# lh3/miniasm

Measured on AMD Instinct MI355X. Metric: PAF overlaps processed/sec (hit-filter->trans-reduce->GFA), higher is better.
Workload: dtype u32

## Files before the change

include/mahip.h:

```cpp
#ifndef MAHIP_H
#define MAHIP_H

#include <stddef.h>
#include <stdint.h>
#include "miniasm_amd.h"

#ifdef __cplusplus
extern "C" {
#endif

typedef struct mahip_ctx mahip_ctx_t;

int mahip_device_count(void);
mahip_ctx_t *mahip_create(int device, void *stream);
void mahip_destroy(mahip_ctx_t *c);
const char *mahip_strerror(void);
int mahip_sync(mahip_ctx_t *c);
int mahip_first_launch(mahip_ctx_t *c);

int mahip_hits_upload(mahip_ctx_t *c, const ma_hit_t *h, size_t n, uint32_t n_seq);
int mahip_hits_adopt(mahip_ctx_t *c, const void *d_hits, size_t n, uint32_t n_seq);
int mahip_set_shard(mahip_ctx_t *c, uint32_t q_beg, uint32_t q_end);
int mahip_hits_balance(mahip_ctx_t *c, int world, uint32_t *bounds);
int mahip_set_shard_bounds(mahip_ctx_t *c, const uint32_t *bounds, int world);
const uint32_t *mahip_shard_bounds(mahip_ctx_t *c, int *world);

typedef struct {
	uint64_t n_lines;
	uint64_t n_records;
	uint64_t n_stored_lines;
	uint64_t n_hits;
	uint64_t name_bytes;
	uint32_t n_seq, max_qs;
	uint32_t n_excl;
} mahip_paf_info_t;
int mahip_paf_load_mem(mahip_ctx_t *c, const void *text, size_t nbytes);
int mahip_paf_load_fd(mahip_ctx_t *c, int fd, size_t nbytes);
int mahip_paf_parse(mahip_ctx_t *c, int min_span, int min_match, int bi_dir, mahip_paf_info_t *info);
int mahip_paf_parse_excl(mahip_ctx_t *c, int min_span, int min_match, int bi_dir, int no_cont, int max_hang, float int_frac, mahip_paf_info_t *info);
int mahip_paf_load_fd_range(mahip_ctx_t *c, int fd, size_t off, size_t nbytes);
int mahip_paf_parse_sharded(mahip_ctx_t *c, int min_span, int min_match, int bi_dir, mahip_paf_info_t *info);
int mahip_hits_route(mahip_ctx_t *c, uint64_t *n_total, uint64_t *bytes_sent);
int mahip_paf_names(mahip_ctx_t *c, char *names, uint32_t *lens);
int mahip_paf_seqs(mahip_ctx_t *c, char *names, void *seqs16, uint64_t *tot_len);
int mahip_paf_release(mahip_ctx_t *c);
uint32_t mahip_paf_max_qs(mahip_ctx_t *c);
int mahip_hits_raw_download(mahip_ctx_t *c, ma_hit_t *out);
int mahip_hits_raw_extract(mahip_ctx_t *c, uint32_t q_beg, uint32_t q_end, void *d_dst, size_t *n_out);
int mahip_hits_raw_extract_pos(mahip_ctx_t *c, uint32_t q_beg, uint32_t q_end, void *d_dst, uint32_t *d_pos, size_t *n_out);
int mahip_hits_set_positions(mahip_ctx_t *c, const uint32_t *pos, int on_device, uint64_t n_total);
int mahip_hits_have_positions(mahip_ctx_t *c);

int mahip_set_hints(mahip_ctx_t *c, uint32_t max_qs);
int mahip_set_run_stride(mahip_ctx_t *c, int stride);
uint64_t mahip_hits_sorted_runs(mahip_ctx_t *c);
int mahip_memcpy_h2d(mahip_ctx_t *c, void *d_dst, const void *h_src, size_t bytes);
int mahip_memcpy_d2h(mahip_ctx_t *c, void *h_dst, const void *d_src, size_t bytes);
int mahip_set_exact_ties(mahip_ctx_t *c, int mode);
typedef struct {
	uint64_t arc_tie_groups;
	uint64_t arc_tie_arcs;
	uint64_t push_conflicts;
	uint64_t hit_ties;
	int arc_walk, hit_walk;
	int unrepaired;
	uint64_t push_conflicts_seen;
	uint64_t hit_walk_reads;
} mahip_tie_info_t;
int mahip_tie_stats(mahip_ctx_t *c, mahip_tie_info_t *out);
int mahip_hits_sort(mahip_ctx_t *c);
int mahip_hits_index(mahip_ctx_t *c);

int mahip_hits_sub(mahip_ctx_t *c, int min_dp, float min_iden, int end_clip, int slot, size_t *n_remained);
int mahip_hits_cut(mahip_ctx_t *c, int slot, int min_span, size_t *n_live);
int mahip_hits_flt(mahip_ctx_t *c, int slot, int max_hang, int min_ovlp, size_t *n_live, float *cov);
int mahip_sub_merge(mahip_ctx_t *c);
int mahip_hits_contained(mahip_ctx_t *c, const ma_opt_t *opt, const uint8_t *seq_del, uint32_t *n_seq_new, size_t *n_live);

int mahip_hits_cutflt_sub(mahip_ctx_t *c, int cut_slot, int min_span, int max_hang, int min_ovlp, int min_dp, float min_iden, int end_clip,
                          int out_slot, size_t *n_cut, size_t *n_flt, float *cov, size_t *n_remained);
int mahip_hits_cut_contained(mahip_ctx_t *c, int cut_slot, int min_span, const ma_opt_t *opt, size_t *n_cut, uint32_t *n_seq_new);
int mahip_hits_cut_contained_flags(mahip_ctx_t *c, int cut_slot, int min_span, const ma_opt_t *opt);
int mahip_hits_cut_contained_finish(mahip_ctx_t *c, size_t *n_cut, uint32_t *n_seq_new);

int mahip_sub_upload(mahip_ctx_t *c, int slot, const ma_sub_t *sub, size_t n_sub);
int mahip_sub_download(mahip_ctx_t *c, int slot, ma_sub_t *sub, int squeezed);
int mahip_seqdel_download(mahip_ctx_t *c, uint8_t *del);
int mahip_map_download(mahip_ctx_t *c, int32_t *map);
uint32_t mahip_n_seq_new(mahip_ctx_t *c);
int mahip_survivors_download(mahip_ctx_t *c, uint32_t *old_ids);
size_t mahip_hits_live(mahip_ctx_t *c);
int mahip_hits_download(mahip_ctx_t *c, ma_hit_t *out, size_t *n);

int mahip_sg_gen(mahip_ctx_t *c, const ma_opt_t *opt, int use_sub, const uint32_t *seq_len, const uint8_t *seq_del, uint32_t *n_arc);
int mahip_asg_upload(mahip_ctx_t *c, const asg_t *g);
int mahip_asg_del_trans(mahip_ctx_t *c, int fuzz, uint32_t *n_reduced);
int mahip_asg_symm(mahip_ctx_t *c, uint32_t *n_multi, uint32_t *n_asymm);
int mahip_asg_del_multi(mahip_ctx_t *c, uint32_t *n_multi);
int mahip_asg_del_asymm(mahip_ctx_t *c, uint32_t *n_asymm);
int mahip_asg_del_short(mahip_ctx_t *c, float drop_ratio, uint32_t *n_short);
int mahip_asg_squeeze(mahip_ctx_t *c);
int mahip_tail_handoff(mahip_ctx_t *from, mahip_ctx_t *to);
int mahip_asg_cut_tip(mahip_ctx_t *c, int max_ext, uint32_t *n_cut);
int mahip_asg_cut_internal(mahip_ctx_t *c, int max_ext, uint32_t *n_cut);
int mahip_asg_cut_biloop(mahip_ctx_t *c, int max_ext, uint32_t *n_cut);
int mahip_asg_pop_bubble(mahip_ctx_t *c, int max_dist, uint32_t *n_pop, uint32_t *n_tips);
uint32_t mahip_bubble_seq_sweeps(mahip_ctx_t *c);
int mahip_ug_gen(mahip_ctx_t *c, uint32_t *n_utg, uint32_t *n_members, uint32_t *n_uarc);
int mahip_ug_download(mahip_ctx_t *c, uint32_t *u_n, uint32_t *u_len, uint32_t *u_start, uint32_t *u_end, uint32_t *u_off, uint64_t *members, asg_arc_t *uarcs);
typedef struct { uint64_t src_off, dst_off; uint32_t src_len, len; uint32_t rev, pad; } mahip_useq_job_t;
int mahip_useq_begin(mahip_ctx_t *c, size_t arena_bytes);
int mahip_useq_batch(mahip_ctx_t *c, const char *h_seq, size_t seq_bytes, const mahip_useq_job_t *h_jobs, size_t n_jobs);
int mahip_useq_end(mahip_ctx_t *c, char *h_arena);
uint32_t mahip_asg_n_arc(mahip_ctx_t *c);
uint64_t mahip_asg_trans_inner(mahip_ctx_t *c);
int mahip_asg_download(mahip_ctx_t *c, asg_t *g);

#define MAHIP_BUF_SUB0  0
#define MAHIP_BUF_SUB1  1
#define MAHIP_BUF_RCONT 2
#define MAHIP_BUF_RUSED 3
#define MAHIP_BUF_SDEL  4
int mahip_copy_out(mahip_ctx_t *c, int which, void *d_dst, size_t first, size_t count);
int mahip_copy_in(mahip_ctx_t *c, int which, const void *d_src, size_t first, size_t count);
int mahip_hits_contained_flags(mahip_ctx_t *c, const ma_opt_t *opt);
int mahip_hits_contained_finish(mahip_ctx_t *c, const uint8_t *seq_del, uint32_t *n_seq_new, size_t *n_live);
int mahip_sg_flags(mahip_ctx_t *c, const ma_opt_t *opt, int use_sub, const uint32_t *seq_len, const uint8_t *seq_del);
int mahip_sg_finish(mahip_ctx_t *c, uint32_t *n_arc);
int mahip_asg_export_rows(mahip_ctx_t *c, void *d_dst);
int mahip_asg_import_rows(mahip_ctx_t *c, const void *d_src, const uint32_t *counts, int n_ranks, size_t stride);
int mahip_set_full_input(mahip_ctx_t *c, int full);
int mahip_sg_push_conflicts(mahip_ctx_t *c, uint64_t *n_conf);
int mahip_sg_push_fix(mahip_ctx_t *c);
int mahip_asg_export_rows_push(mahip_ctx_t *c, void *d_dst);
int mahip_asg_import_push_rows(mahip_ctx_t *c, const void *d_src, const uint32_t *counts, int n_ranks, size_t stride);
int mahip_asg_del_trans_range(mahip_ctx_t *c, int fuzz, uint32_t v_beg, uint32_t v_end, uint32_t *n_reduced);
int mahip_asg_flags_out(mahip_ctx_t *c, void *d_dst, size_t first, size_t count);
int mahip_asg_flags_in(mahip_ctx_t *c, const void *d_src, size_t first, size_t count);
int mahip_asg_cleanup(mahip_ctx_t *c, uint32_t *n_arc);

int mahip_comm_unique_id(void *id128);
int mahip_comm_init(mahip_ctx_t *c, const void *id128, int rank, int world);
int mahip_comm_init_shm(mahip_ctx_t *c, const char *name, int rank, int world);
void mahip_comm_destroy(mahip_ctx_t *c);
int mahip_comm_rank(mahip_ctx_t *c);
int mahip_comm_world(mahip_ctx_t *c);
int mahip_comm_active(mahip_ctx_t *c);
int mahip_comm_all_gather(mahip_ctx_t *c, const void *d_send, void *d_recv, size_t bytes_per_rank);
int mahip_comm_all_reduce_max_u8(mahip_ctx_t *c, void *d_buf, size_t n);
int mahip_comm_all_reduce_sum_u64(mahip_ctx_t *c, uint64_t *h_vals, size_t n);
typedef struct {
	void *user;
	int (*all_gather)(void *user, const void *send, void *recv, size_t bytes);
	int (*all_reduce_max_u8)(void *user, void *buf, size_t n);
	int (*all_reduce_sum_u64)(void *user, uint64_t *vals, size_t n);
	int (*all_reduce_sum_u32)(void *user, void *buf, size_t n);
	int (*all_to_all_v)(void *user, const void *send, void *recv, const uint64_t *bytes);
} mahip_comm_ext_t;
int mahip_comm_init_ext(mahip_ctx_t *c, int rank, int world, const mahip_comm_ext_t *ext);
int mahip_comm_all_reduce_sum_u32(mahip_ctx_t *c, void *d_buf, size_t n);
int mahip_comm_all_to_all_v(mahip_ctx_t *c, const void *d_send, void *d_recv, const uint64_t *bytes);
int mahip_comm_all_gather_u64(mahip_ctx_t *c, const uint64_t *h_vals, size_t n, uint64_t *h_out);
int mahip_comm_barrier(mahip_ctx_t *c);
int mahip_xbuf(mahip_ctx_t *c, int slot, size_t bytes, void **d_ptr);

int mahip_prof_enable(mahip_ctx_t *c, int enable);
int mahip_prof_reset(mahip_ctx_t *c);
typedef struct { const char *name; uint64_t launches; double total_ms; double alg_bytes; } mahip_prof_t;
int mahip_prof_get(mahip_ctx_t *c, mahip_prof_t *out, int max);
int mahip_mark(mahip_ctx_t *c, int slot);
int mahip_marks_ms(mahip_ctx_t *c, int first, int n, float *ms);
size_t mahip_mem_bytes(mahip_ctx_t *c);
size_t mahip_mem_pool_bytes(mahip_ctx_t *c);
int mahip_mem_trim(mahip_ctx_t *c, size_t *released);

int mahip_diag_patterns(void);
const char *mahip_diag_name(int pattern);
int mahip_diag_run(mahip_ctx_t *c, int pattern, size_t bytes, int reps, double *best_ms, double *moved);
#define MAHIP_PTR_SUB0    0
#define MAHIP_PTR_SUB1    1
#define MAHIP_PTR_RDFLAG  2
void *mahip_devptr(mahip_ctx_t *c, int which, size_t *bytes);

#ifdef __cplusplus
}
#endif
#endif
```

miniasm_amd/csrc/graph.hip:

```cpp
#include "mahip_internal.hpp"
#include <type_traits>

#define DEAD 0x80000000u
#define ADEL 0x80000000u

struct HitColsG { const uint32_t *qid, *qs, *qe, *tn, *ts, *te, *ml, *bl; };
struct ArcCols { uint32_t *u, *v, *len, *ol; };

static HitColsG gcols_of(mahip_ctx *c)
{
	HitColsG h;
	h.qid = P<uint32_t>(c->col[0]); h.qs = P<uint32_t>(c->col[1]); h.qe = P<uint32_t>(c->col[2]); h.tn = P<uint32_t>(c->col[3]);
	h.ts = P<uint32_t>(c->col[4]); h.te = P<uint32_t>(c->col[5]); h.ml = P<uint32_t>(c->col[6]); h.bl = P<uint32_t>(c->col[7]);
	return h;
}
static ArcCols arcs_of(mahip_ctx *c, int g)
{
	ArcCols a;
	a.u = P<uint32_t>(c->au[g]); a.v = P<uint32_t>(c->av[g]); a.len = P<uint32_t>(c->alen[g]); a.ol = P<uint32_t>(c->aol[g]);
	return a;
}
static int reserve_arcs(mahip_ctx *c, size_t n)
{
	for (int g = 0; g < 2; ++g) {
		CHK(dev_reserve(c, c->au[g], (n + 4) * 4)); CHK(dev_reserve(c, c->av[g], (n + 4) * 4));
		CHK(dev_reserve(c, c->alen[g], (n + 4) * 4)); CHK(dev_reserve(c, c->aol[g], (n + 4) * 4));
	}
	CHK(dev_reserve(c, c->keep, (n + 16) * 4)); CHK(dev_reserve(c, c->pos, (n + 16) * 4));
	return 0;
}

__global__ __launch_bounds__(256) void k_sg_seq(const uint2 *__restrict__ sub, const uint8_t *__restrict__ r_del, const uint32_t *__restrict__ seq_len,
                                                 const uint8_t *__restrict__ seq_del, uint32_t n_seq, uint32_t *__restrict__ slen, uint8_t *__restrict__ sdel)
{
	uint32_t r = blockIdx.x * 256 + threadIdx.x;
	if (r >= n_seq) return;
	uint32_t len; int del;
	if (sub) { uint2 s = sub[r]; len = s.y - (s.x & 0x7fffffffu); del = s.x >> 31; }
	else len = seq_len[r], del = 0;
	if (seq_del) del |= seq_del[r];
	if (r_del) del |= r_del[r];
	slen[r] = len; sdel[r] = (uint8_t)del;
}

#define SG_TILE 16384u

__device__ __forceinline__ int sg_candidate(const HitColsG &h, size_t i, const uint32_t *__restrict__ slen, int max_hang, float int_frac, int min_ovlp,
                                            const uint8_t *__restrict__ lazy_del, mc_arc_t *x, uint32_t *q_, uint32_t *t_, int *self_rc)
{
	const uint32_t q = h.qid[i];
	if (lazy_del && lazy_del[q]) return -100;
	if (h.bl[i] & DEAD) return -100;
	const uint32_t t = h.tn[i];
	if (lazy_del && lazy_del[t]) return -100;
	uint32_t qs = h.qs[i], qe = h.qe[i], ts = h.ts[i], te = h.te[i];
	int rev = h.ml[i] >> 31;
	*q_ = q; *t_ = t;
	*self_rc = q == t && qs == ts && qe == te && rev;
	return mc_hit2arc(q, qs, qe, t, ts, te, rev, (int)slen[q], (int)slen[t], max_hang, int_frac, min_ovlp, x);
}

__global__ __launch_bounds__(256) void k_sg_arcs(HitColsG h, size_t n, const uint32_t *__restrict__ slen, uint8_t *__restrict__ sdel,
                                                  int max_hang, float int_frac, int min_ovlp, unsigned long long *__restrict__ ctr, const uint8_t *__restrict__ lazy_del,
                                                  unsigned long long *__restrict__ cmask)
{
	uint32_t mx = 0, n_live = 0;
	for (size_t base = (size_t)blockIdx.x * 256; base < n; base += (size_t)gridDim.x * 256) {
		const size_t i = base + threadIdx.x;
		int cand = 0;
		if (i < n) {
			mc_arc_t x;
			uint32_t q = 0, t = 0;
			int self_rc = 0, r = sg_candidate(h, i, slen, max_hang, int_frac, min_ovlp, lazy_del, &x, &q, &t, &self_rc);
			if (r != -100) {
				++n_live;
				if (r >= 0) {
					if (q == t) { if (self_rc) sdel[q] = 1; }
					else cand = 1, mx = x.len > mx ? x.len : mx;
				} else if (r == MC_HT_QCONT) sdel[q] = 1;
			}
		}
		const unsigned long long m = wv_ballot(cand);
		if ((threadIdx.x & 63) == 0) cmask[i >> 6] = m;
	}
	blk_max_u64(&ctr[CT_MAXLEN], mx);
	blk_add_u64(&ctr[CT_LIVE], n_live);
}

#ifndef SG_DENSE
#define SG_DENSE 6
#endif
__device__ __forceinline__ unsigned long long wv_bcast_u64(unsigned long long x, int src) { return (unsigned long long)__shfl((uint32_t)(x >> 32), src, 64) << 32 | __shfl((uint32_t)x, src, 64); }

__global__ __launch_bounds__(256) void k_sg_emit(HitColsG h, size_t n, const uint32_t *__restrict__ slen, const uint8_t *__restrict__ sdel,
                                                  int max_hang, float int_frac, int min_ovlp, const unsigned long long *cmask,
                                                  uint32_t *__restrict__ tile_cnt, const uint32_t *__restrict__ tile_off, ArcCols out, uint32_t *__restrict__ aslot,
                                                  uint32_t *__restrict__ wpos, unsigned long long *kmask)
{
	__shared__ uint32_t s_w[4];
	const unsigned lane = threadIdx.x & 63;
	const size_t w = (size_t)blockIdx.x * 256 + threadIdx.x, n_words = (n + 63) >> 6, w0 = w - lane;
	unsigned long long m = w < n_words ? cmask[w] : 0ull, kept = 0;
	uint32_t cnt = 0;
	const bool dense = __popcll(m) >= SG_DENSE;
	const unsigned long long dense_lanes = wv_ballot(dense);
	for (unsigned long long dl = dense_lanes; dl; dl &= dl - 1) {
		const int l = __ffsll((long long)dl) - 1;
		const unsigned long long ml = wv_bcast_u64(m, l);
		const size_t i = ((w0 + (size_t)l) << 6) + lane;
		const int k = (ml >> lane & 1ull) && i < n && !sdel[h.qid[i]] && !sdel[h.tn[i]];
		const unsigned long long kb = wv_ballot(k);
		if ((int)lane == l) kept = kb, cnt = (uint32_t)__popcll(kb);
	}
	if (!dense)
		for (unsigned long long rest = m; rest; rest &= rest - 1) {
			const int b = __ffsll((long long)rest) - 1;
			const size_t i = (w << 6) + (size_t)b;
			if (i < n && !sdel[h.qid[i]] && !sdel[h.tn[i]]) kept |= 1ull << b, ++cnt;
		}
	uint32_t tot, ex = block_excl_scan_256(cnt, s_w, &tot);
	if (!out.u) { if (threadIdx.x == 0) tile_cnt[blockIdx.x] = tot; return; }
	uint32_t p = tile_off[blockIdx.x] + ex;
	if (wpos && w < n_words) { wpos[w] = p; kmask[w] = kept; }
	for (unsigned long long dl = dense_lanes; dl; dl &= dl - 1) {
		const int l = __ffsll((long long)dl) - 1;
		const unsigned long long kl = wv_bcast_u64(kept, l);
		const uint32_t pl = __shfl(p, l, 64);
		if (kl >> lane & 1ull) {
			const size_t i = ((w0 + (size_t)l) << 6) + lane;
			const uint32_t pp = pl + (uint32_t)__popcll(kl & wv_lt(lane));
			mc_arc_t x;
			uint32_t q = 0, t = 0;
			int self_rc = 0;
			sg_candidate(h, i, slen, max_hang, int_frac, min_ovlp, nullptr, &x, &q, &t, &self_rc);
			out.u[pp] = x.u; out.v[pp] = x.v; out.len[pp] = x.len; out.ol[pp] = x.ol;
			if (aslot) aslot[pp] = (uint32_t)i;
		}
	}
	if (!dense)
		for (; kept; kept &= kept - 1, ++p) {
			const size_t i = (w << 6) + (size_t)(__ffsll((long long)kept) - 1);
			mc_arc_t x;
			uint32_t q = 0, t = 0;
			int self_rc = 0;
			sg_candidate(h, i, slen, max_hang, int_frac, min_ovlp, nullptr, &x, &q, &t, &self_rc);
			out.u[p] = x.u; out.v[p] = x.v; out.len[p] = x.len; out.ol[p] = x.ol;
			if (aslot) aslot[p] = (uint32_t)i;
		}
}

__global__ __launch_bounds__(256) void k_arc_keep(ArcCols a, size_t n, const uint8_t *__restrict__ sdel, uint32_t *__restrict__ keep, int use_keep_in)
{
	size_t i = (size_t)blockIdx.x * 256 + threadIdx.x;
	if (i >= n) return;
	int k = use_keep_in ? (int)keep[i] : 1;
	if (k) k = !(a.ol[i] & ADEL) && !sdel[a.u[i] >> 1] && !sdel[a.v[i] >> 1];
	keep[i] = k;
}

__global__ __launch_bounds__(256) void k_arc_compact(ArcCols in, size_t n, const uint32_t *__restrict__ keep, const uint32_t *__restrict__ pos, ArcCols out)
{
	size_t i = (size_t)blockIdx.x * 256 + threadIdx.x;
	if (i < n && keep[i]) {
		uint32_t p = pos[i];
		out.u[p] = in.u[i]; out.v[p] = in.v[i]; out.len[p] = in.len[i]; out.ol[p] = in.ol[i];
	}
}

#define RM_ITEMS 8
#define RM_TILE (256 * RM_ITEMS)
#define RMC_ITEMS 8
#define RMC_TILE (256 * RMC_ITEMS)
#define RMC_TILES 16u
#define RMC_GROUP ((size_t)RMC_TILES * RMC_TILE)
__global__ __launch_bounds__(256) void k_arc_rm_count(const uint32_t *__restrict__ aol, size_t n, uint32_t *__restrict__ cnt)
{
	__shared__ uint32_t s_wave[4];
	const size_t g0 = (size_t)blockIdx.x * RMC_GROUP, g1 = g0 + RMC_GROUP < n ? g0 + RMC_GROUP : n;
	uint32_t mine = 0;
	for (size_t b0 = g0; b0 < g1; b0 += 8 * 1024) {
		uint4 w[8];
#pragma unroll
		for (int j = 0; j < 8; ++j) { const size_t b4 = b0 + (size_t)j * 1024 + (size_t)threadIdx.x * 4; w[j] = b4 + 4 <= g1 ? *(const uint4*)(aol + b4) : make_uint4(ADEL, ADEL, ADEL, ADEL); }
#pragma unroll
		for (int j = 0; j < 8; ++j) {
			const size_t b4 = b0 + (size_t)j * 1024 + (size_t)threadIdx.x * 4;
			mine += !(w[j].x & ADEL) + !(w[j].y & ADEL) + !(w[j].z & ADEL) + !(w[j].w & ADEL);
			if (b4 < g1 && b4 + 4 > g1) for (size_t i = b4; i < g1; ++i) mine += !(aol[i] & ADEL);
		}
	}
	uint32_t gtot;
	(void)block_excl_scan_256(mine, s_wave, &gtot);
	if (threadIdx.x == 0) cnt[blockIdx.x] = gtot;
}
__global__ __launch_bounds__(256) void k_arc_rm_write(ArcCols in, size_t n, ArcCols out, const uint32_t *__restrict__ pre)
{
	__shared__ uint32_t s_wave[4];
	const size_t g0 = (size_t)blockIdx.x * RMC_GROUP, g1 = g0 + RMC_GROUP < n ? g0 + RMC_GROUP : n;
	uint32_t p0 = pre[blockIdx.x];
	for (size_t tb = g0; tb < g1; tb += RMC_TILE) {
		const size_t base = tb + (size_t)threadIdx.x * RMC_ITEMS;
		uint32_t ol[RMC_ITEMS], keep = 0;
		if (base + RMC_ITEMS <= n) {
			const uint4 *po = (const uint4*)(in.ol + base);
			const uint4 c0 = po[0], c1 = po[1];
			ol[0] = c0.x, ol[1] = c0.y, ol[2] = c0.z, ol[3] = c0.w, ol[4] = c1.x, ol[5] = c1.y, ol[6] = c1.z, ol[7] = c1.w;
		} else {
#pragma unroll
			for (int i = 0; i < RMC_ITEMS; ++i) ol[i] = base + i < n ? in.ol[base + i] : ADEL;
		}
#pragma unroll
		for (int i = 0; i < RMC_ITEMS; ++i) if (!(ol[i] & ADEL)) keep |= 1u << i;
		uint32_t tot;
		const uint32_t ex = block_excl_scan_256((uint32_t)__popc(keep), s_wave, &tot);
		uint32_t p = p0 + ex;
#pragma unroll
		for (int i = 0; i < RMC_ITEMS; ++i)
			if (keep >> i & 1u) { out.u[p] = in.u[base + i]; out.v[p] = in.v[base + i]; out.len[p] = in.len[base + i]; out.ol[p] = ol[i]; ++p; }
		p0 += tot;
	}
}

__global__ __launch_bounds__(256) void k_arc_rm_chain(ArcCols in, size_t n, const uint8_t *__restrict__ sdel, ArcCols out, uint32_t *__restrict__ d_total,
                                                       unsigned long long *state, uint32_t *ticket, uint32_t ticket_base, uint32_t epoch)
{
	__shared__ uint32_t s_wave[4];
	__shared__ uint32_t s_tile, s_prefix;
	if (threadIdx.x == 0) s_tile = atomicAdd(ticket, 1u) - ticket_base;
	__syncthreads();
	const uint32_t tile = s_tile;
	const size_t base = (size_t)tile * RM_TILE + (size_t)threadIdx.x * RM_ITEMS;
	uint32_t u[RM_ITEMS], v[RM_ITEMS], ol[RM_ITEMS], keep = 0;
	if (base + RM_ITEMS <= n) {
		const uint4 *pu = (const uint4*)(in.u + base), *pv = (const uint4*)(in.v + base), *po = (const uint4*)(in.ol + base);
		const uint4 a0 = pu[0], a1 = pu[1], b0 = pv[0], b1 = pv[1], c0 = po[0], c1 = po[1];
		u[0] = a0.x, u[1] = a0.y, u[2] = a0.z, u[3] = a0.w, u[4] = a1.x, u[5] = a1.y, u[6] = a1.z, u[7] = a1.w;
// ... 540 lines not shown
				if (mark[y] == 2) aol[st + i] |= ADEL, ++cnt;
				mark[y] = 0;
			}
			if (cnt) atomicAdd(&ctr[CT_NRED], (unsigned long long)cnt);
		}
		__syncthreads();
	}
	blk_add_u64(&ctr[CT_TRINNER], n_inner);
}

__global__ __launch_bounds__(256) void k_asg_multi(ArcCols a, size_t n, const unsigned long long *__restrict__ idx, unsigned long long *__restrict__ ctr)
{
	uint32_t cnt = 0;
	for (size_t e = (size_t)blockIdx.x * 256 + threadIdx.x; e < n; e += (size_t)gridDim.x * 256) {
		uint32_t st = (uint32_t)(idx[a.u[e]] >> 32), v = a.v[e];
		int del = 0;
		for (uint32_t j = st; j < e; ++j) if (a.v[j] == v) { del = 1; break; }
		if (del) a.ol[e] |= ADEL, ++cnt;
	}
	blk_add_u64(&ctr[CT_NMULTI], cnt);
}

__global__ __launch_bounds__(256) void k_asg_asymm(ArcCols a, size_t n, const unsigned long long *__restrict__ idx, unsigned long long *__restrict__ ctr)
{
	uint32_t cnt = 0;
	uint64_t probed = 0;
	for (size_t e = (size_t)blockIdx.x * 256 + threadIdx.x; e < n; e += (size_t)gridDim.x * 256) {
		uint32_t v = a.v[e] ^ 1, u = a.u[e] ^ 1;
		unsigned long long x = idx[v];
		uint32_t st = (uint32_t)(x >> 32), nv = (uint32_t)x, i;
		for (i = 0; i < nv; ++i) if (a.v[st + i] == u) break;
		probed += i < nv ? i + 1 : nv;
		if (i == nv) a.ol[e] |= ADEL, ++cnt;
	}
	blk_add_u64(&ctr[CT_NASYMM], cnt);
	blk_add_u64(&ctr[CT_PROBED], probed);
}

__global__ __launch_bounds__(256) void k_asg_short(ArcCols a, const unsigned long long *__restrict__ idx, uint32_t n_vtx, float drop_ratio, unsigned long long *__restrict__ ctr)
{
	uint32_t cnt = 0;
	for (uint32_t v = blockIdx.x * 256 + threadIdx.x; v < n_vtx; v += gridDim.x * 256) {
		unsigned long long x = idx[v];
		uint32_t st = (uint32_t)(x >> 32), nv = (uint32_t)x;
		if (nv >= 2) {
			float p = (float)(int32_t)(a.ol[st] & 0x7fffffffu) * drop_ratio;
			uint32_t thres = (uint32_t)((double)p + .499), i;
			for (i = nv - 1; i >= 1 && (a.ol[st + i] & 0x7fffffffu) < thres; --i);
			for (i = i + 1; i < nv; ++i) a.ol[st + i] |= ADEL, ++cnt;
		}
	}
	blk_add_u64(&ctr[CT_NSHORT], cnt);
}

__global__ __launch_bounds__(256) void k_arc_from_aos(const asg_arc_t *__restrict__ in, size_t n, ArcCols a)
{
	size_t i = (size_t)blockIdx.x * 256 + threadIdx.x;
	if (i < n) { uint4 r = *(const uint4*)(in + i); a.len[i] = r.x; a.u[i] = r.y; a.v[i] = r.z; a.ol[i] = r.w; }
}
__global__ __launch_bounds__(256) void k_seq_from_aos(const uint32_t *__restrict__ seq, uint32_t n_seq, uint32_t *__restrict__ slen, uint8_t *__restrict__ sdel)
{
	uint32_t r = blockIdx.x * 256 + threadIdx.x;
	if (r < n_seq) { uint32_t x = seq[r]; slen[r] = x & 0x7fffffffu; sdel[r] = (uint8_t)(x >> 31); }
}
__global__ __launch_bounds__(256) void k_arc_to_aos(ArcCols a, size_t n, const int32_t *__restrict__ map, asg_arc_t *__restrict__ out)
{
	size_t i = (size_t)blockIdx.x * 256 + threadIdx.x;
	if (i >= n) return;
	uint32_t u = a.u[i], v = a.v[i];
	if (map) u = (uint32_t)map[u >> 1] << 1 | (u & 1), v = (uint32_t)map[v >> 1] << 1 | (v & 1);
	*(uint4*)(out + i) = make_uint4(a.len[i], u, v, a.ol[i]);
}
__global__ __launch_bounds__(256) void k_seq_to_aos(const uint32_t *__restrict__ slen, const uint8_t *__restrict__ sdel, const unsigned long long *__restrict__ idx,
                                                     const int32_t *__restrict__ map, uint32_t n_seq, uint32_t *__restrict__ seq, unsigned long long *__restrict__ idx_out)
{
	uint32_t r = blockIdx.x * 256 + threadIdx.x;
	if (r >= n_seq) return;
	int32_t m = map ? map[r] : (int32_t)r;
	if (m < 0) return;
	seq[m] = (slen[r] & 0x7fffffffu) | (uint32_t)sdel[r] << 31;
	idx_out[2 * (size_t)m] = idx[2 * (size_t)r]; idx_out[2 * (size_t)m + 1] = idx[2 * (size_t)r + 1];
}


__global__ __launch_bounds__(256) void k_arc_rows_out(ArcCols a, size_t n, uint4 *__restrict__ rows)
{
	size_t i = (size_t)blockIdx.x * 256 + threadIdx.x;
	if (i < n) rows[i] = make_uint4(a.u[i], a.v[i], a.len[i], a.ol[i]);
}
__global__ __launch_bounds__(256) void k_arc_rows_in(const uint4 *__restrict__ rows, size_t n, size_t dst0, ArcCols a)
{
	size_t i = (size_t)blockIdx.x * 256 + threadIdx.x;
	if (i < n) { uint4 r = rows[i]; a.u[dst0 + i] = r.x; a.v[dst0 + i] = r.y; a.len[dst0 + i] = r.z; a.ol[dst0 + i] = r.w; }
}

__global__ __launch_bounds__(256) void k_rows_permute(const uint4 *__restrict__ in, size_t n, const uint32_t *__restrict__ perm, uint4 *__restrict__ out)
{
	size_t i = (size_t)blockIdx.x * 256 + threadIdx.x;
	if (i < n) out[i] = in[perm[i]];
}

uint32_t graph_nseq(const mahip_ctx *c) { return c->gsq ? c->n_seq_new : c->n_seq; }
static const int32_t *graph_map(mahip_ctx *c) { return c->has_map && !c->gsq ? (const int32_t*)P<int32_t>(c->map) : (const int32_t*)nullptr; }

static int arc_reindex(mahip_ctx *c)
{
	size_t V = 2 * (size_t)graph_nseq(c);
	CHK(dev_reserve(c, c->idx, (V + 2) * 8));
	HIPCHK(hipMemsetAsync(c->idx.p, 0, V * 8, c->st));
	if (c->n_arc) {
		ProfScope ps(c, "k_arc_index", 16.0 * (double)c->n_arc);
		hipLaunchKernelGGL(k_arc_index, dim3(grid_for(c->n_arc, 256)), dim3(256), 0, c->st, (const uint32_t*)P<uint32_t>(c->au[c->ag]), (size_t)c->n_arc, P<unsigned long long>(c->idx));
	}
	HIPCHK(hipGetLastError());
	return 0;
}

static int arc_cleanup(mahip_ctx *c, size_t n_in, int keep_in, int index_mode)
{
	uint32_t *d_tot = (uint32_t*)(P<unsigned long long>(c->ctr) + CT_TOTAL);
	if (n_in == 0) { c->n_arc = 0; return index_mode < 0 ? 0 : arc_reindex(c); }
	ArcCols in = arcs_of(c, c->ag), out = arcs_of(c, c->ag ^ 1);
	if (!keep_in) {
		ProfScope ps(c, "k_arc_rm", 32.0 * (double)n_in);
		if (c->arcs_clean) {
			const size_t ng = (n_in + RMC_GROUP - 1) / RMC_GROUP;
			hipLaunchKernelGGL(k_arc_rm_count, dim3((unsigned)ng), dim3(256), 0, c->st, (const uint32_t*)in.ol, n_in, P<uint32_t>(c->keep));
			CHK(scan_exclusive_u32(c, P<uint32_t>(c->keep), P<uint32_t>(c->pos), ng, d_tot));
			hipLaunchKernelGGL(k_arc_rm_write, dim3((unsigned)ng), dim3(256), 0, c->st, in, n_in, out, (const uint32_t*)P<uint32_t>(c->pos));
		} else {
			const size_t nb = (n_in + RM_TILE - 1) / RM_TILE;
			uint32_t *ticket; unsigned long long *state; uint32_t ticket_base, epoch;
			CHK(scan_chain_begin(c, nb, &state, &ticket, &ticket_base, &epoch));
			hipLaunchKernelGGL(k_arc_rm_chain, dim3((unsigned)nb), dim3(256), 0, c->st, in, n_in, (const uint8_t*)P<uint8_t>(c->sdel), out, d_tot, state, ticket, ticket_base, epoch);
		}
	} else {
		ProfScope ps(c, "k_arc_rm", 32.0 * (double)n_in);
		hipLaunchKernelGGL(k_arc_keep, dim3(grid_for(n_in, 256)), dim3(256), 0, c->st, in, n_in, (const uint8_t*)P<uint8_t>(c->sdel), P<uint32_t>(c->keep), keep_in);
		CHK(scan_exclusive_u32(c, P<uint32_t>(c->keep), P<uint32_t>(c->pos), n_in, d_tot));
		hipLaunchKernelGGL(k_arc_compact, dim3(grid_for(n_in, 256)), dim3(256), 0, c->st, in, n_in, (const uint32_t*)P<uint32_t>(c->keep), (const uint32_t*)P<uint32_t>(c->pos), out);
	}
	CHK(ctr_fetch(c));
	uint32_t n_out = (uint32_t)(c->h_ctr[CT_TOTAL] & 0xffffffffu);
	c->ag ^= 1;
	int changed = n_out != n_in;
	c->n_arc = n_out;
	c->arcs_clean = true;
	if (index_mode > 0 || (index_mode == 0 && changed)) CHK(arc_reindex(c));
	return 0;
}

static int bitlen_u64(uint64_t x) { int b = 0; while (x) ++b, x >>= 1; return b; }

extern "C" int mahip_sg_flags(mahip_ctx_t *c, const ma_opt_t *opt, int use_sub, const uint32_t *seq_len, const uint8_t *seq_del)
{
	HIPCHK(hipSetDevice(c->dev));
	CHK(hits_need_cols(c, "mahip_sg_gen"));
	size_t n = c->n_hits;
	uint32_t R = c->n_seq;
	CHK(dev_reserve(c, c->slen, ((size_t)R + 4) * 4)); CHK(dev_reserve(c, c->sdel, (size_t)R + 16));
	c->sg_max_hang = opt->max_hang; c->sg_int_frac = opt->int_frac; c->sg_min_ovlp = opt->min_ovlp;
	c->gsq = false; c->arcs_clean = false;
	CHK(ctr_zero(c));
	unsigned long long *ctr = P<unsigned long long>(c->ctr);
	const uint32_t *d_len = nullptr; const uint8_t *d_del = nullptr;
	if (seq_len) { CHK(dev_reserve(c, c->big0, ((size_t)R + 4) * 4)); HIPCHK(hipMemcpyAsync(c->big0.p, seq_len, (size_t)R * 4, hipMemcpyHostToDevice, c->st)); d_len = P<uint32_t>(c->big0); }
	if (seq_del) { CHK(dev_reserve(c, c->big1, (size_t)R + 16)); HIPCHK(hipMemcpyAsync(c->big1.p, seq_del, R, hipMemcpyHostToDevice, c->st)); d_del = P<uint8_t>(c->big1); }
	if (!use_sub && !d_len) { mahip_set_error("mahip_sg_gen: need sub or seq_len"); return -1; }
	if (R) hipLaunchKernelGGL(k_sg_seq, dim3(grid_for(R, 256)), dim3(256), 0, c->st, use_sub ? (const uint2*)P<uint2>(c->sub[0]) : (const uint2*)nullptr,
	                          c->has_map ? (const uint8_t*)P<uint8_t>(c->r_del) : (const uint8_t*)nullptr, d_len, d_del, R, P<uint32_t>(c->slen), P<uint8_t>(c->sdel));
	c->ag = 0;
	if (n) CHK(dev_reserve(c, c->sgmask, (n / 64 + 8) * 8));
	if (n) {
		ProfScope ps(c, "k_sg_arcs", 64.0 * (double)c->n_live);
		hipLaunchKernelGGL(k_sg_arcs, dim3(grid_for(n, 256, MA_STREAM_BLOCKS)), dim3(256), 0, c->st, gcols_of(c), n, (const uint32_t*)P<uint32_t>(c->slen), P<uint8_t>(c->sdel),
		                   opt->max_hang, opt->int_frac, opt->min_ovlp, ctr,
		                   c->lazy_squeeze ? (const uint8_t*)P<uint8_t>(c->r_del) : (const uint8_t*)nullptr, P<unsigned long long>(c->sgmask));
	}
	HIPCHK(hipGetLastError());
	return 0;
}

static int push_stable_order(mahip_ctx *c, size_t m, int *gen, uint64_t *conflicts)
{
	unsigned long long *ctr = P<unsigned long long>(c->ctr);
	const int bs = hits_qs_bits(c);
	int bq = 0;
	for (uint64_t x = c->n_seq ? c->n_seq - 1 : 0xffffffffull; x; x >>= 1) ++bq;
	for (int k = 0; k < 2; ++k) { CHK(dev_reserve(c, c->key[k], (m + 1) * 8)); CHK(dev_reserve(c, c->val[k], (m + 1) * 4)); }
	hipLaunchKernelGGL(k_arc_slot_keys, dim3(grid_for(m, 256)), dim3(256), 0, c->st, (const uint32_t*)P<uint32_t>(c->aslot), m, c->d_aos, (const uint32_t*)P<uint32_t>(c->sidx),
	                   P<uint64_t>(c->key[0]), P<uint32_t>(c->val[0]));
	*gen = 0;
	CHK(radix_sort_pairs(c, m, 0, bs, 32, 32 + (bq ? bq : 1), gen));
	HIPCHK(hipMemsetAsync(ctr + ST_PUSH_CONFLICTS, 0, 8, c->st));
	hipLaunchKernelGGL(k_arc_push_conflicts, dim3(grid_for(m, 256, MA_STREAM_BLOCKS)), dim3(256), 0, c->st, (const uint64_t*)P<uint64_t>(c->key[*gen]), m, ctr);
	CHK(ctr_fetch(c));
	*conflicts = c->h_ctr[ST_PUSH_CONFLICTS];
	return 0;
}

static int push_order(mahip_ctx *c, size_t m, bool exact, int *gen, const ArcCols *pushed = nullptr, const ArcCols *sorted = nullptr)
{
	uint64_t conf = 0;
	bool want_known = false;
	TieLaps tl(c);
	CHK(push_stable_order(c, m, gen, &conf));
	tl.lap("stable push order + conflicts");
	c->tie.push_conflicts = conf;
	c->tie.push_conflicts_seen = conf;
	static const bool filter_on = !(getenv("MA_TIE_NO_FILTER") && atoi(getenv("MA_TIE_NO_FILTER")) != 0);
	if (exact && conf && pushed && sorted && filter_on && m < 0xffffffffull) {
		unsigned long long *ctr = P<unsigned long long>(c->ctr);
		const int32_t *map = c->has_map ? (const int32_t*)P<int32_t>(c->map) : (const int32_t*)nullptr;
		uint64_t *S = P<uint64_t>(c->key[*gen ^ 1]);
		CHK(dev_reserve(c, c->keep, (m + 16) * 4)); CHK(dev_reserve(c, c->pos, (m + 16) * 4));
		hipLaunchKernelGGL(k_arc_keys_ref, dim3(grid_for(m, 256)), dim3(256), 0, c->st, *sorted, m, map, S);
		hipLaunchKernelGGL(k_tie_pair_flags, dim3(grid_for(m, 256)), dim3(256), 0, c->st, (const uint64_t*)S, m, P<uint32_t>(c->keep));
		CHK(scan_exclusive_u32(c, P<uint32_t>(c->keep), P<uint32_t>(c->pos), m, nullptr));
		HIPCHK(hipMemsetAsync(ctr + ST_PUSH_SEEN, 0, 8, c->st));
		const size_t want_bytes = ((size_t)c->n_seq / 32 + 2) * 4;
		CHK(dev_reserve(c, c->wantb, want_bytes));
		HIPCHK(hipMemsetAsync(c->wantb.p, 0, want_bytes, c->st));
		hipLaunchKernelGGL(k_arc_push_conflicts_seen, dim3(grid_for(m, 256, MA_STREAM_BLOCKS)), dim3(256), 0, c->st, (const uint64_t*)P<uint64_t>(c->key[*gen]), (const uint32_t*)P<uint32_t>(c->val[*gen]),
		                   *pushed, map, (const uint64_t*)S, (const uint32_t*)P<uint32_t>(c->pos), (uint32_t)m, ctr, P<uint32_t>(c->wantb));
		CHK(ctr_fetch(c));
		c->tie.push_conflicts_seen = c->h_ctr[ST_PUSH_SEEN];
		want_known = true;
		tl.lap("conflicts the arc sort can see");
	}
	if (exact && c->tie.push_conflicts_seen) {
		const int g_keep = *gen; (void)g_keep;
		static const bool walk_all = getenv("MA_TIE_WALK_ALL") && atoi(getenv("MA_TIE_WALK_ALL")) != 0;
		CHK(hits_reference_rank(c, false, want_known && !walk_all));
		for (int k = 0; k < 2; ++k) { CHK(dev_reserve(c, c->key[k], (m + 1) * 8)); CHK(dev_reserve(c, c->val[k], (m + 1) * 4)); }
		hipLaunchKernelGGL(k_arc_push_keys, dim3(grid_for(m, 256)), dim3(256), 0, c->st, (const uint32_t*)P<uint32_t>(c->aslot), (const uint32_t*)P<uint32_t>(c->hrank), m,
		                   P<uint64_t>(c->key[0]), P<uint32_t>(c->val[0]));
		*gen = 0;
		int bh = 0;
		for (uint64_t x = c->n_in; x; x >>= 1) ++bh;
		CHK(radix_sort_pairs(c, m, 0, bh ? bh : 1, 0, 0, gen));
	}
	return 0;
}

extern "C" int mahip_sg_finish(mahip_ctx_t *c, uint32_t *n_arc)
{
	HIPCHK(hipSetDevice(c->dev));
	size_t n = c->n_hits;
	uint32_t R = c->n_seq;
	CHK(ctr_fetch(c));
	c->n_live = (size_t)c->h_ctr[CT_LIVE];
	if (c->prof) prof_patch_last(c, "k_sg_arcs", 64.0 * (double)c->n_live);
	c->n_arc = 0; c->ag = 0;
	const bool sharded = c->q_beg > 0 || (c->n_seq && c->q_end < c->n_seq);
	const bool want_slots = c->sorted_here && c->sidx.p != nullptr;
	const int blen = bitlen_u64(c->h_ctr[CT_MAXLEN]);
	{ const uint64_t keep_hit_ties = c->tie.hit_ties; const int keep_walk = c->hrank_ready; memset(&c->tie, 0, sizeof(c->tie)); c->tie.hit_ties = keep_hit_ties; c->tie.hit_walk = keep_walk; }
	if (n) {
		const size_t n_tiles = (n + SG_TILE - 1) / SG_TILE;
		const unsigned long long *lazy = (const unsigned long long*)P<unsigned long long>(c->sgmask);
		uint32_t *d_tot = (uint32_t*)(P<unsigned long long>(c->ctr) + CT_TOTAL);
		ArcCols none = { nullptr, nullptr, nullptr, nullptr };
		CHK(dev_reserve(c, c->keep, (n + 16) * 4)); CHK(dev_reserve(c, c->pos, (n + 16) * 4));
		{
			ProfScope ps(c, "k_sg_emit", 4.0 * (double)n + 64.0 * (double)c->n_live);
			hipLaunchKernelGGL(k_sg_emit, dim3((unsigned)n_tiles), dim3(256), 0, c->st, gcols_of(c), n, (const uint32_t*)P<uint32_t>(c->slen), (const uint8_t*)P<uint8_t>(c->sdel),
			                   c->sg_max_hang, c->sg_int_frac, c->sg_min_ovlp, lazy, P<uint32_t>(c->keep), (const uint32_t*)nullptr, none, (uint32_t*)nullptr, (uint32_t*)nullptr, (unsigned long long*)nullptr);
		}
		CHK(scan_exclusive_u32(c, P<uint32_t>(c->keep), P<uint32_t>(c->pos), n_tiles, d_tot));
		CHK(ctr_fetch(c));
		c->n_arc = (uint32_t)(c->h_ctr[CT_TOTAL] & 0xffffffffu);
		CHK(reserve_arcs(c, c->n_arc));
		if (want_slots) CHK(dev_reserve(c, c->aslot, ((size_t)c->n_arc + 4) * 4));
		CHK(dev_reserve(c, c->apos, (n / 64 + 8) * 4));
		if (c->n_arc) {
			ProfScope ps(c, "k_sg_emit", 4.0 * (double)n + 64.0 * (double)c->n_live + 16.0 * (double)c->n_arc);
			hipLaunchKernelGGL(k_sg_emit, dim3((unsigned)n_tiles), dim3(256), 0, c->st, gcols_of(c), n, (const uint32_t*)P<uint32_t>(c->slen), (const uint8_t*)P<uint8_t>(c->sdel),
			                   c->sg_max_hang, c->sg_int_frac, c->sg_min_ovlp, lazy, (uint32_t*)nullptr, (const uint32_t*)P<uint32_t>(c->pos), arcs_of(c, 0),
			                   want_slots ? P<uint32_t>(c->aslot) : (uint32_t*)nullptr, P<uint32_t>(c->apos), P<unsigned long long>(c->sgmask));
		}
	} else CHK(reserve_arcs(c, 0));
	c->n_push = 0; c->push_ordered = false;
	if (sharded && c->tie_mode != 0) {
		CHK(dev_reserve(c, c->pushrows[0], ((size_t)c->n_arc + 1) * 16));
		if (c->n_arc) hipLaunchKernelGGL(k_arc_rows_out, dim3(grid_for(c->n_arc, 256)), dim3(256), 0, c->st, arcs_of(c, c->ag), (size_t)c->n_arc, (uint4*)c->pushrows[0].p);
		c->n_push = c->n_arc;
	}
	if (c->n_arc > 1) {
		size_t m = c->n_arc;
		for (int k = 0; k < 2; ++k) { CHK(dev_reserve(c, c->key[k], (m + 1) * 8)); CHK(dev_reserve(c, c->val[k], (m + 1) * 4)); }
		ArcCols in = arcs_of(c, c->ag), out = arcs_of(c, c->ag ^ 1);
		unsigned long long *ctr = P<unsigned long long>(c->ctr);
		const int32_t *map = c->has_map ? (const int32_t*)P<int32_t>(c->map) : (const int32_t*)nullptr;
		int gen = 0, need_walk = c->tie_mode == 1 && !sharded;
		TieLaps tl(c);
		if (c->tie_mode == 0 && want_slots) {
			int g0 = 0;
			CHK(push_order(c, m, false, &g0));
			hipLaunchKernelGGL(k_arc_permute, dim3(grid_for(m, 256)), dim3(256), 0, c->st, in, m, (const uint32_t*)P<uint32_t>(c->val[g0]), out);
			c->ag ^= 1;
			in = arcs_of(c, c->ag); out = arcs_of(c, c->ag ^ 1);
		}
		bool idx_done = false;
		if (c->tie_mode != 1 || sharded) {
			bool fast = blen + AG_IB + 1 <= 31 && !getenv("MA_ARC_RADIX");
			if (fast) {
				const size_t V = 2 * (size_t)R;
				const uint32_t q_lo = sharded ? c->q_beg : 0u, q_hi = sharded && c->q_end < R ? c->q_end : R, Rr = q_hi > q_lo ? q_hi - q_lo : 1;
				CHK(dev_reserve(c, c->idx, (V + 2) * 8));
				HIPCHK(hipMemsetAsync(c->idx.p, 0, V * 8, c->st));
				HIPCHK(hipMemsetAsync(ctr + CT_OVF2, 0, 8, c->st));
				HIPCHK(hipMemsetAsync(ctr + CT_STICKY, 0, (64 - CT_STICKY) * 8, c->st));
				{
					ProfScope ps(c, "k_arc_group_sort", 48.0 * (double)m);
					const unsigned grid = grid_for(((size_t)Rr + 63) / 64, 4, MA_STREAM_BLOCKS);
					const uint32_t *goff = (const uint32_t*)P<uint32_t>(c->goff), *wpos = (const uint32_t*)P<uint32_t>(c->apos);
					const unsigned long long *km = (const unsigned long long*)P<unsigned long long>(c->sgmask);
					hipLaunchKernelGGL(k_arc_group_sort<true>, dim3(grid), dim3(256), 0, c->st, in, out, goff, wpos, km, (uint32_t)n, (uint32_t)m, q_lo, q_hi, blen ? blen : 1, P<unsigned long long>(c->idx), ctr);
					hipLaunchKernelGGL(k_arc_group_sort<false>, dim3(grid), dim3(256), 0, c->st, in, out, goff, wpos, km, (uint32_t)n, (uint32_t)m, q_lo, q_hi, blen ? blen : 1, P<unsigned long long>(c->idx), ctr);
				}
				CHK(ctr_fetch(c));
				if (c->h_ctr[CT_OVF2]) fast = false;
				else {
					idx_done = true;
					if (c->tie_mode == 2 && !sharded) {
						c->tie.arc_tie_groups = c->h_ctr[ST_ARC_TIE_GROUPS]; c->tie.arc_tie_arcs = c->h_ctr[ST_ARC_TIE_ARCS];
						need_walk = c->tie.arc_tie_groups > 0;
					}
				}
			}
			if (!fast) {
			hipLaunchKernelGGL(k_arc_keys, dim3(grid_for(m, 256)), dim3(256), 0, c->st, in, m, P<uint64_t>(c->key[0]), P<uint32_t>(c->val[0]));
// ... 443 lines not shown
```

Measured before the change: 6.283 billion.

## Add per-read grouped arc flag kernel that skips deleted reads' hit ranges

Adds k_sg_arcs_by_read, which walks reads in wavefront chunks and processes only the hit ranges of reads not lazily deleted, using the goff group offsets from sorted hits. The host picks it automatically when hits are grouped over the whole input, lazy squeeze is on, and at most a quarter of reads survive. The goal is to avoid scanning hits that belong to deleted reads. In exchange it adds a memset of the mask, atomicOr on partially covered mask words, and per-read serialisation within a wave. A probe entry point is also added for testing.

```diff
diff --git a/include/mahip.h b/include/mahip.h
--- a/include/mahip.h
+++ b/include/mahip.h
@@ -127,6 +127,8 @@
 int mahip_hits_contained_finish(mahip_ctx_t *c, const uint8_t *seq_del, uint32_t *n_seq_new, size_t *n_live);
 int mahip_sg_flags(mahip_ctx_t *c, const ma_opt_t *opt, int use_sub, const uint32_t *seq_len, const uint8_t *seq_del);
 int mahip_sg_finish(mahip_ctx_t *c, uint32_t *n_arc);
+int mahip_sg_flags_probe(mahip_ctx_t *c, const ma_opt_t *opt, int use_sub, const uint32_t *seq_len, const uint8_t *seq_del, int form, const uint8_t *read_del,
+                         uint64_t *cmask, uint8_t *sdel, uint64_t *out3);
 int mahip_asg_export_rows(mahip_ctx_t *c, void *d_dst);
 int mahip_asg_import_rows(mahip_ctx_t *c, const void *d_src, const uint32_t *counts, int n_ranks, size_t stride);
 int mahip_set_full_input(mahip_ctx_t *c, int full);
diff --git a/miniasm_amd/csrc/graph.hip b/miniasm_amd/csrc/graph.hip
--- a/miniasm_amd/csrc/graph.hip
+++ b/miniasm_amd/csrc/graph.hip
@@ -45,11 +45,9 @@
 
 #define SG_TILE 16384u
 
-__device__ __forceinline__ int sg_candidate(const HitColsG &h, size_t i, const uint32_t *__restrict__ slen, int max_hang, float int_frac, int min_ovlp,
-                                            const uint8_t *__restrict__ lazy_del, mc_arc_t *x, uint32_t *q_, uint32_t *t_, int *self_rc)
-{
-	const uint32_t q = h.qid[i];
-	if (lazy_del && lazy_del[q]) return -100;
+__device__ __forceinline__ int sg_candidate_of(const HitColsG &h, size_t i, uint32_t q, const uint32_t *__restrict__ slen, int max_hang, float int_frac, int min_ovlp,
+                                               const uint8_t *__restrict__ lazy_del, mc_arc_t *x, uint32_t *q_, uint32_t *t_, int *self_rc)
+{
 	if (h.bl[i] & DEAD) return -100;
 	const uint32_t t = h.tn[i];
 	if (lazy_del && lazy_del[t]) return -100;
@@ -58,6 +56,14 @@
 	*q_ = q; *t_ = t;
 	*self_rc = q == t && qs == ts && qe == te && rev;
 	return mc_hit2arc(q, qs, qe, t, ts, te, rev, (int)slen[q], (int)slen[t], max_hang, int_frac, min_ovlp, x);
+}
+
+__device__ __forceinline__ int sg_candidate(const HitColsG &h, size_t i, const uint32_t *__restrict__ slen, int max_hang, float int_frac, int min_ovlp,
+                                            const uint8_t *__restrict__ lazy_del, mc_arc_t *x, uint32_t *q_, uint32_t *t_, int *self_rc)
+{
+	const uint32_t q = h.qid[i];
+	if (lazy_del && lazy_del[q]) return -100;
+	return sg_candidate_of(h, i, q, slen, max_hang, int_frac, min_ovlp, lazy_del, x, q_, t_, self_rc);
 }
 
 __global__ __launch_bounds__(256) void k_sg_arcs(HitColsG h, size_t n, const uint32_t *__restrict__ slen, uint8_t *__restrict__ sdel,
@@ -82,6 +88,51 @@
 		}
 		const unsigned long long m = wv_ballot(cand);
 		if ((threadIdx.x & 63) == 0) cmask[i >> 6] = m;
+	}
+	blk_max_u64(&ctr[CT_MAXLEN], mx);
+	blk_add_u64(&ctr[CT_LIVE], n_live);
+}
+
+__global__ __launch_bounds__(256) void k_sg_arcs_by_read(HitColsG h, size_t n, const uint32_t *__restrict__ goff, uint32_t n_seq, const uint32_t *__restrict__ slen,
+                                                          uint8_t *__restrict__ sdel, int max_hang, float int_frac, int min_ovlp, unsigned long long *__restrict__ ctr,
+                                                          const uint8_t *__restrict__ lazy_del, unsigned long long *__restrict__ cmask)
+{
+	const unsigned lane = threadIdx.x & 63;
+	const uint32_t n_chunks = (uint32_t)(((size_t)n_seq + 63) >> 6);
+	uint32_t mx = 0, n_live = 0;
+	for (uint32_t ch = blockIdx.x * 4 + (threadIdx.x >> 6); ch < n_chunks; ch += gridDim.x * 4) {
+		const size_t q = (size_t)ch * 64 + lane;
+		size_t g0 = 0, g1 = 0;
+		if (q < n_seq && !(lazy_del && lazy_del[q])) {
+			g0 = goff[q]; g1 = goff[q + 1];
+			if (g1 > n) g1 = n;
+		}
+		for (unsigned long long todo = wv_ballot(g0 < g1); todo; todo &= todo - 1) {
+			const int l = __ffsll((long long)todo) - 1;
+			const size_t s0 = wv_bcast((uint32_t)g0, l), s1 = wv_bcast((uint32_t)g1, l);
+			const uint32_t qr = ch * 64 + (uint32_t)l;
+			for (size_t base = s0 & ~(size_t)63; base < s1; base += 64) {
+				const size_t i = base + lane;
+				int cand = 0;
+				if (i >= s0 && i < s1) {
+					mc_arc_t x;
+					uint32_t qq = 0, t = 0;
+					int self_rc = 0, r = sg_candidate_of(h, i, qr, slen, max_hang, int_frac, min_ovlp, lazy_del, &x, &qq, &t, &self_rc);
+					if (r != -100) {
+						++n_live;
+						if (r >= 0) {
+							if (qr == t) { if (self_rc) sdel[qr] = 1; }
+							else cand = 1, mx = x.len > mx ? x.len : mx;
+						} else if (r == MC_HT_QCONT) sdel[qr] = 1;
+					}
+				}
+				const unsigned long long m = wv_ballot(cand);
+				if (lane == 0 && m) {
+					if (base >= s0 && base + 64 <= s1) cmask[base >> 6] = m;
+					else atomicOr(&cmask[base >> 6], m);
+				}
+			}
+		}
 	}
 	blk_max_u64(&ctr[CT_MAXLEN], mx);
 	blk_add_u64(&ctr[CT_LIVE], n_live);
@@ -928,7 +979,8 @@
 
 static int bitlen_u64(uint64_t x) { int b = 0; while (x) ++b, x >>= 1; return b; }
 
-extern "C" int mahip_sg_flags(mahip_ctx_t *c, const ma_opt_t *opt, int use_sub, const uint32_t *seq_len, const uint8_t *seq_del)
+#define FLAGS_OWN ((const uint8_t*)1)
+static int sg_flags(mahip_ctx *c, const ma_opt_t *opt, int use_sub, const uint32_t *seq_len, const uint8_t *seq_del, int form, const uint8_t *d_lazy, int *by_read_out)
 {
 	HIPCHK(hipSetDevice(c->dev));
 	CHK(hits_need_cols(c, "mahip_sg_gen"));
@@ -946,14 +998,47 @@
 	if (R) hipLaunchKernelGGL(k_sg_seq, dim3(grid_for(R, 256)), dim3(256), 0, c->st, use_sub ? (const uint2*)P<uint2>(c->sub[0]) : (const uint2*)nullptr,
 	                          c->has_map ? (const uint8_t*)P<uint8_t>(c->r_del) : (const uint8_t*)nullptr, d_len, d_del, R, P<uint32_t>(c->slen), P<uint8_t>(c->sdel));
 	c->ag = 0;
+	if (d_lazy == FLAGS_OWN) d_lazy = c->lazy_squeeze ? (const uint8_t*)P<uint8_t>(c->r_del) : (const uint8_t*)nullptr;
+	const bool grouped = c->sorted_here && R && !(c->q_beg > 0 || c->q_end < R) && n < 0xffffffffull;
+	if (form == 1 && !grouped) { mahip_set_error("mahip_sg_flags: the per-read form needs hits grouped by mahip_hits_sort on the whole input"); return -1; }
+	const bool by_read = form == 1 || (form < 0 && grouped && d_lazy && c->has_map && (uint64_t)c->n_seq_new * 4 <= R);
+	if (by_read_out) *by_read_out = by_read;
 	if (n) CHK(dev_reserve(c, c->sgmask, (n / 64 + 8) * 8));
 	if (n) {
 		ProfScope ps(c, "k_sg_arcs", 64.0 * (double)c->n_live);
+		if (by_read) {
+			HIPCHK(hipMemsetAsync(c->sgmask.p, 0, (n / 64 + 1) * 8, c->st));
+			hipLaunchKernelGGL(k_sg_arcs_by_read, dim3(grid_for(((size_t)R + 63) / 64, 4, MA_STREAM_BLOCKS)), dim3(256), 0, c->st, gcols_of(c), n, (const uint32_t*)P<uint32_t>(c->goff), R,
+			                   (const uint32_t*)P<uint32_t>(c->slen), P<uint8_t>(c->sdel), opt->max_hang, opt->int_frac, opt->min_ovlp, ctr, d_lazy, P<unsigned long long>(c->sgmask));
+		} else
 		hipLaunchKernelGGL(k_sg_arcs, dim3(grid_for(n, 256, MA_STREAM_BLOCKS)), dim3(256), 0, c->st, gcols_of(c), n, (const uint32_t*)P<uint32_t>(c->slen), P<uint8_t>(c->sdel),
-		                   opt->max_hang, opt->int_frac, opt->min_ovlp, ctr,
-		                   c->lazy_squeeze ? (const uint8_t*)P<uint8_t>(c->r_del) : (const uint8_t*)nullptr, P<unsigned long long>(c->sgmask));
+		                   opt->max_hang, opt->int_frac, opt->min_ovlp, ctr, d_lazy, P<unsigned long long>(c->sgmask));
 	}
 	HIPCHK(hipGetLastError());
+	return 0;
+}
+
+extern "C" int mahip_sg_flags(mahip_ctx_t *c, const ma_opt_t *opt, int use_sub, const uint32_t *seq_len, const uint8_t *seq_del)
+{
+	return sg_flags(c, opt, use_sub, seq_len, seq_del, -1, FLAGS_OWN, nullptr);
+}
+
+extern "C" int mahip_sg_flags_probe(mahip_ctx_t *c, const ma_opt_t *opt, int use_sub, const uint32_t *seq_len, const uint8_t *seq_del, int form, const uint8_t *read_del,
+                                    uint64_t *cmask, uint8_t *sdel, uint64_t *out3)
+{
+	const uint8_t *d_lazy = FLAGS_OWN;
+	int by_read = 0;
+	if (read_del) {
+		HIPCHK(hipSetDevice(c->dev));
+		CHK(dev_reserve(c, c->wseg, (size_t)c->n_seq + 16));
+		HIPCHK(hipMemcpyAsync(c->wseg.p, read_del, c->n_seq, hipMemcpyHostToDevice, c->st));
+		d_lazy = (const uint8_t*)c->wseg.p;
+	}
+	CHK(sg_flags(c, opt, use_sub, seq_len, seq_del, form, d_lazy, &by_read));
+	CHK(ctr_fetch(c));
+	if (cmask && c->n_hits) HIPCHK(hipMemcpy(cmask, c->sgmask.p, ((c->n_hits + 63) / 64) * 8, hipMemcpyDeviceToHost));
+	if (sdel && c->n_seq) HIPCHK(hipMemcpy(sdel, c->sdel.p, c->n_seq, hipMemcpyDeviceToHost));
+	if (out3) { out3[0] = c->h_ctr[CT_LIVE]; out3[1] = c->h_ctr[CT_MAXLEN]; out3[2] = (uint64_t)by_read; }
 	return 0;
 }
 
```

Result: faster. 6.412 billion (median of 6 runs) (+2.1%).

## Walk hits per query group in sg_arcs to skip deleted reads' hits

Applied to the files above, without the earlier changes.

Adds a grouped variant of the arc-candidate kernel that runs when hits are sorted by query. Each wave takes a chunk of 64 query ids, reads their hit ranges from goff, skips queries with no hits or that are lazily deleted, and scans only the remaining ranges without reloading qid per hit. Ranges are not 64-aligned, so candidate bits are merged into a pre-zeroed mask with atomicOr, which adds a memset and atomics. Load balance may suffer when queries have very uneven hit counts or many queries have only a few hits.

```diff
diff --git a/miniasm_amd/csrc/graph.hip b/miniasm_amd/csrc/graph.hip
--- a/miniasm_amd/csrc/graph.hip
+++ b/miniasm_amd/csrc/graph.hip
@@ -45,11 +45,9 @@
 
 #define SG_TILE 16384u
 
-__device__ __forceinline__ int sg_candidate(const HitColsG &h, size_t i, const uint32_t *__restrict__ slen, int max_hang, float int_frac, int min_ovlp,
-                                            const uint8_t *__restrict__ lazy_del, mc_arc_t *x, uint32_t *q_, uint32_t *t_, int *self_rc)
-{
-	const uint32_t q = h.qid[i];
-	if (lazy_del && lazy_del[q]) return -100;
+__device__ __forceinline__ int sg_candidate_q(const HitColsG &h, size_t i, uint32_t q, const uint32_t *__restrict__ slen, int max_hang, float int_frac, int min_ovlp,
+                                              const uint8_t *__restrict__ lazy_del, mc_arc_t *x, uint32_t *q_, uint32_t *t_, int *self_rc)
+{
 	if (h.bl[i] & DEAD) return -100;
 	const uint32_t t = h.tn[i];
 	if (lazy_del && lazy_del[t]) return -100;
@@ -58,6 +56,13 @@
 	*q_ = q; *t_ = t;
 	*self_rc = q == t && qs == ts && qe == te && rev;
 	return mc_hit2arc(q, qs, qe, t, ts, te, rev, (int)slen[q], (int)slen[t], max_hang, int_frac, min_ovlp, x);
+}
+__device__ __forceinline__ int sg_candidate(const HitColsG &h, size_t i, const uint32_t *__restrict__ slen, int max_hang, float int_frac, int min_ovlp,
+                                            const uint8_t *__restrict__ lazy_del, mc_arc_t *x, uint32_t *q_, uint32_t *t_, int *self_rc)
+{
+	const uint32_t q = h.qid[i];
+	if (lazy_del && lazy_del[q]) return -100;
+	return sg_candidate_q(h, i, q, slen, max_hang, int_frac, min_ovlp, lazy_del, x, q_, t_, self_rc);
 }
 
 __global__ __launch_bounds__(256) void k_sg_arcs(HitColsG h, size_t n, const uint32_t *__restrict__ slen, uint8_t *__restrict__ sdel,
@@ -82,6 +87,50 @@
 		}
 		const unsigned long long m = wv_ballot(cand);
 		if ((threadIdx.x & 63) == 0) cmask[i >> 6] = m;
+	}
+	blk_max_u64(&ctr[CT_MAXLEN], mx);
+	blk_add_u64(&ctr[CT_LIVE], n_live);
+}
+
+#define SGA_CHUNK 64u
+__global__ __launch_bounds__(256) void k_sg_arcs_grp(HitColsG h, const uint32_t *__restrict__ goff, uint32_t n_seq, const uint32_t *__restrict__ slen, uint8_t *__restrict__ sdel,
+                                                      int max_hang, float int_frac, int min_ovlp, unsigned long long *__restrict__ ctr, const uint8_t *__restrict__ lazy_del,
+                                                      unsigned long long *__restrict__ cmask)
+{
+	const unsigned lane = threadIdx.x & 63, wave = threadIdx.x >> 6;
+	uint32_t mx = 0, n_live = 0;
+	for (uint64_t qb = (uint64_t)(blockIdx.x * 4 + wave) * SGA_CHUNK; qb < n_seq; qb += (uint64_t)gridDim.x * 4 * SGA_CHUNK) {
+		const bool in = qb + lane < n_seq;
+		const uint32_t beg_l = in ? goff[qb + lane] : 0, end_l = in ? goff[qb + lane + 1] : 0;
+		const int del_l = in && lazy_del ? lazy_del[qb + lane] : 0;
+		unsigned long long todo = wv_ballot(in && end_l > beg_l && !del_l);
+		while (todo) {
+			const int qbit = __ffsll((long long)todo) - 1;
+			todo &= todo - 1;
+			const uint32_t q = (uint32_t)qb + (uint32_t)qbit;
+			const uint32_t beg = __shfl(beg_l, qbit, 64), end = __shfl(end_l, qbit, 64);
+			for (uint32_t s = beg; s < end; s += 64) {
+				const uint32_t i = s + lane;
+				int cand = 0;
+				if (i < end) {
+					mc_arc_t x;
+					uint32_t q_ = 0, t = 0;
+					int self_rc = 0, r = sg_candidate_q(h, i, q, slen, max_hang, int_frac, min_ovlp, lazy_del, &x, &q_, &t, &self_rc);
+					if (r != -100) {
+						++n_live;
+						if (r >= 0) {
+							if (q == t) { if (self_rc) sdel[q] = 1; }
+							else cand = 1, mx = x.len > mx ? x.len : mx;
+						} else if (r == MC_HT_QCONT) sdel[q] = 1;
+					}
+				}
+				const unsigned long long m = wv_ballot(cand);
+				const unsigned sh = s & 63u;
+				if (m && lane == 0) atomicOr(&cmask[s >> 6], m << sh);
+				if (m && lane == 1 && sh && (m >> (64u - sh))) atomicOr(&cmask[(s >> 6) + 1], m >> (64u - sh));
+				if (end - s <= 64u) break;
+			}
+		}
 	}
 	blk_max_u64(&ctr[CT_MAXLEN], mx);
 	blk_add_u64(&ctr[CT_LIVE], n_live);
@@ -949,9 +998,14 @@
 	if (n) CHK(dev_reserve(c, c->sgmask, (n / 64 + 8) * 8));
 	if (n) {
 		ProfScope ps(c, "k_sg_arcs", 64.0 * (double)c->n_live);
+		const uint8_t *lazy = c->lazy_squeeze ? (const uint8_t*)P<uint8_t>(c->r_del) : (const uint8_t*)nullptr;
+		if (c->sorted_here && R) {
+			HIPCHK(hipMemsetAsync(c->sgmask.p, 0, ((n + 63) / 64) * 8, c->st));
+			hipLaunchKernelGGL(k_sg_arcs_grp, dim3(grid_for(R, 4 * SGA_CHUNK, MA_STREAM_BLOCKS)), dim3(256), 0, c->st, gcols_of(c), (const uint32_t*)P<uint32_t>(c->goff), R,
+			                   (const uint32_t*)P<uint32_t>(c->slen), P<uint8_t>(c->sdel), opt->max_hang, opt->int_frac, opt->min_ovlp, ctr, lazy, P<unsigned long long>(c->sgmask));
+		} else
 		hipLaunchKernelGGL(k_sg_arcs, dim3(grid_for(n, 256, MA_STREAM_BLOCKS)), dim3(256), 0, c->st, gcols_of(c), n, (const uint32_t*)P<uint32_t>(c->slen), P<uint8_t>(c->sdel),
-		                   opt->max_hang, opt->int_frac, opt->min_ovlp, ctr,
-		                   c->lazy_squeeze ? (const uint8_t*)P<uint8_t>(c->r_del) : (const uint8_t*)nullptr, P<unsigned long long>(c->sgmask));
+		                   opt->max_hang, opt->int_frac, opt->min_ovlp, ctr, lazy, P<unsigned long long>(c->sgmask));
 	}
 	HIPCHK(hipGetLastError());
 	return 0;
```

Result: slower. 6.561 billion before, 6.259 billion after (-4.6%).
